# weiquan/salt

Measured on AMD Instinct MI355X. Metric: Mreads/s aligned (100 bp SE, GRCh38+snp144) at 1/2/4/8 MI355X vs CPU ref, higher is better.
Workload: dtype u32; 1 GPU; GRCh38-scale synthetic (SURVEY 8d config 3 = BASELINE configs[2]): 3100000000 bp genome in 24 contigs, 14800000 SNPs, k=21, 1000000 x 100 bp SE reads per GPU per step, 8 distinct resident batches rotated, inputs and results resident in HBM; read_len=100, distinct_batches=8, options=default (-s 50 -m 1000, overlap = k), streams_per_gpu=4

## Files before the change

salt_amd/csrc/salt_align.hip:

```cpp
#include <type_traits>
#include "salt_device.h"
#include "salt_kernels.h"

namespace salt {

#define WSYNC() do { __builtin_amdgcn_fence(__ATOMIC_ACQ_REL, "wavefront"); __builtin_amdgcn_wave_barrier(); \
                     __builtin_amdgcn_fence(__ATOMIC_ACQ_REL, "wavefront"); } while (0)

static constexpr int MAXL = SALT_MAX_READ_LEN;
static constexpr int SLOTS = SALT_MAX_SEED_SLOTS;
static constexpr int MAXLOC = SALT_MAX_LOCATE;
static constexpr int LVK = 31;
static_assert(offsetof(salt_result_t, strand) == 4 && offsetof(salt_result_t, mapq) == 7 && offsetof(salt_result_t, b0) == 8 &&
              offsetof(salt_result_t, b1) == 12 && offsetof(salt_result_t, seq_start) == 16 && offsetof(salt_result_t, seq_end) == 18 &&
              offsetof(salt_result_t, n_hits) == 20 && offsetof(salt_result_t, n_cigar) == 22 && offsetof(salt_result_t, skipped) == 23 &&
              offsetof(salt_result_t, hits) == 24 && sizeof(salt_hit_t) == 8, "salt_result_t header layout");
static constexpr int NHIT = 6;
__device__ __forceinline__ uint32_t mapq_quot(uint32_t x, uint32_t b0)
{
    const uint32_t v = 255u * x;
    return b0 == 1u ? v : b0 == 2u ? v / 2u : b0 == 3u ? v / 3u : v / b0;
}
static constexpr uint32_t INF = 255;

// ... 922 lines not shown
            for (uint32_t k = 0; k < 8; ++k) {
                if (!mm) break;
                const uint32_t bit = (uint32_t)__ffsll((long long)mm) - 1u;
                if (k == q) c = b + bit;
                mm &= mm - 1;
            }
            m = mm;
            const bool act = c != 0xFFFFFFFFu;
            uint32_t pos = act ? cand[c] : 0u;
            if (pos >= ref_len) pos = 0xFFFFFFFFu;
            u32x4_a4 x = { 0u, 0u, 0u, 0u };
            if (act && need && pos != 0xFFFFFFFFu) x = *reinterpret_cast<const u32x4_a4 *>(ref + (pos >> 3) + 4 * sub);
            const uint32_t mism = quad_mismatch<8>(x, pos, pmw, nvalid);
            if (act && sub == 0) out[c] = (uint8_t)((mism > 3 || pos == 0xFFFFFFFFu) ? INF : mism);
        }
    }
}

__device__ __forceinline__ uint32_t popc(uint32_t m) { return (uint32_t)__popc(m); }
__device__ __forceinline__ uint32_t popc(uint64_t m) { return (uint32_t)__popcll(m); }
__device__ __forceinline__ int first_bit(uint32_t m) { return __ffs((int)m) - 1; }
__device__ __forceinline__ int first_bit(uint64_t m) { return __ffsll((long long)m) - 1; }
template <int GW> struct LaneGroup {
    static_assert(GW == 64 || GW == 32, "a wave or half of one");
    typedef std::conditional_t<GW == 64, uint64_t, uint32_t> mask_t;
    static __device__ __forceinline__ uint32_t lane() { return lane_id() & (uint32_t)(GW - 1); }
    static __device__ __forceinline__ mask_t ballot(bool x)
    {
        const uint64_t m = __ballot(x);
        if constexpr (GW == 64) return m; else return (lane_id() & 32u) ? (uint32_t)(m >> 32) : (uint32_t)m;
    }
    static __device__ __forceinline__ uint32_t bcast(uint32_t v, int src)
    {
        if constexpr (GW == 64) return (uint32_t)__builtin_amdgcn_readlane((int)v, src);
        else return (uint32_t)__shfl((int)v, (int)(lane_id() & 32u) + src);
    }
    static __device__ __forceinline__ mask_t below() { return ((mask_t)1 << lane()) - (mask_t)1; }
    static __device__ __forceinline__ uint32_t sum(uint32_t v)
    {
        for (int o = GW / 2; o > 0; o >>= 1) v += (uint32_t)__shfl_xor((int)v, o);
        return v;
    }
};

template <int LN = 4, int GW = 64>
__device__ __forceinline__ void verify_quads_2(const uint32_t *__restrict__ ref, uint32_t ref_len, const uint32_t *pm0, const uint32_t *pm1, uint32_t L,
                                               const uint32_t *c0, uint32_t n0, const uint32_t *c1, uint32_t n1, uint8_t *o0, uint8_t *o1)
{
    constexpr uint32_t CPW = (uint32_t)GW / LN;
    const uint32_t lane = LaneGroup<GW>::lane(), sub = lane & (uint32_t)(LN - 1), q = lane / (uint32_t)LN;
    const uint32_t nw = (L + 7) >> 3, n = n0 + n1;
    const uint32_t nvalid = L > 32u * sub ? (L - 32u * sub < 32u ? L - 32u * sub : 32u) : 0u;
    const bool behind = LN == 8 && GW == 32 && !(4u * sub < nw + 1u);
    uint32_t pa[4], pb[4];
#pragma unroll
    for (int t = 0; t < 4; ++t) { const bool in = (4 * sub + t) < nw; pa[t] = in ? pm0[4 * sub + t] : 0u; pb[t] = in ? pm1[4 * sub + t] : 0u; }
    for (uint32_t b = 0; b < n; b += 4u * CPW) {
        uint32_t pos[4]; u32x4_a4 x[4]; bool act[4], rev[4];
// ... 868 lines not shown
        uint32_t strand, pos, k;
        if (which == 0) { strand = out->strand; pos = out->pos; k = out->n_diff; }
        else {
            const uint32_t h = which - 1, n0 = out->n_hits[0];
            strand = h >= n0; const uint32_t j = strand ? h - n0 : h;
            pos = out->hits[strand][j].pos; k = out->hits[strand][j].n_diff;
        }
        for (uint32_t t = lane; t < (L + 7) >> 3; t += 64) w.pm[strand][t] = rec[strand * ap.pg.nw8 + t];
        WSYNC();
        lv_cigar(ix.ref, w, lvtab + blockIdx.x, (int)strand, L, pos, (int)k);
        uint16_t *dst = which == 0 ? out->cigar : out->hit_cigar[which - 1];
        if (lane < (uint32_t)w.n_cig) dst[lane] = w.cig[lane];
        if (lane == 0) { if (which == 0) out->n_cigar = (uint8_t)w.n_cig; else out->hit_n_cigar[which - 1] = (uint8_t)w.n_cig; }
        WSYNC();
    }
}

__host__ __device__ __forceinline__ uint32_t qseg_cap(uint32_t n_reads) { return n_reads / QUEUE_RANGES + 8u; }
__device__ __forceinline__ void queue_push(uint32_t *__restrict__ qseg, QueueRange *__restrict__ ranges, uint32_t n_reads, uint32_t r)
{
    const uint32_t s = (r >> 2) & (QUEUE_RANGES - 1u);
    qseg[(size_t)s * qseg_cap(n_reads) + atomicAdd(&ranges[s].push, 1u)] = r;
}
__global__ void __launch_bounds__(256)
k_queue_pack(const uint32_t *__restrict__ qseg, const QueueRange *__restrict__ ranges, uint32_t n_reads, uint32_t *__restrict__ queue, SeCtl *__restrict__ ctl)
{
    __shared__ uint32_t base_s, cnt_s;
    if (threadIdx.x == 0) {
        uint32_t base = 0, total = 0;
        for (uint32_t s = 0; s < QUEUE_RANGES; ++s) { const uint32_t c = ranges[s].push; if (s < blockIdx.x) base += c; total += c; }
        base_s = base; cnt_s = ranges[blockIdx.x].push;
        if (blockIdx.x == 0) ctl->light_queued = total;
    }
    __syncthreads();
    const uint32_t *src = qseg + (size_t)blockIdx.x * qseg_cap(n_reads);
    for (uint32_t i = threadIdx.x; i < cnt_s; i += 256) queue[base_s + i] = src[i];
}

static constexpr int LT_LOCI = 128;
static constexpr int LT_MAXL = 160;
static constexpr int L2_SLOTS = 8;

template <int SLOTS, int PMW> struct LightRec {
    uint32_t pm[2][PMW];
    uint32_t sp[4][SLOTS], off[4][SLOTS];
    uint32_t pre[4][SLOTS + 1];
    uint32_t loci[2][LT_LOCI];
    uint32_t hit_pos[2][NHIT];
    uint8_t  hit_nd[2][NHIT];
    uint8_t  val[2][LT_LOCI];
};
template <int GW> using LightLds = LightRec<GW / 4, GW == 64 ? LT_MAXL / 8 : 32>;

template <int GW, int LN, bool INSTR>
__device__ __forceinline__ void light_read(const IndexView &ix, const AlignParams &ap, const uint32_t *__restrict__ pm,
                                           const uint4 *__restrict__ sai_c, const uint4 *__restrict__ sai_r, salt_result_t *__restrict__ results,
                                           uint32_t *__restrict__ queue , QueueRange *__restrict__ ranges,
                                           unsigned long long *__restrict__ ctr, LightLds<GW> &w, const uint32_t r)
{
    typedef LaneGroup<GW> G;
    typedef typename G::mask_t mask_t;
    constexpr uint32_t SLOTS = GW / 4, HALF = GW / 2;
    constexpr uint32_t LMAX = LN == 4 ? 120u : LN == 8 ? 248u : (uint32_t)LT_MAXL;
    static_assert(LMAX <= 8 * sizeof(w.pm[0]) / 4 && (LN != 0 || LMAX <= 248u), "the read fits the record and the window check");
    const uint32_t lane = G::lane();
    const mask_t lt = G::below();
    const uint32_t *rec = pm + (uint64_t)r * ap.pg.pm_stride;
    const uint32_t L = rec[2 * ap.pg.nw8];
    bool heavy = L > LMAX || L < (uint32_t)ap.l_seed || ap.spr > SLOTS || ap.max_locate < 2 * 64;
    uint32_t c_sa_c = 0, c_sa_r = 0, c_verify = 0, c_loci = 0;
    const bool prof = INSTR && ctr && (r & 127u) == 0;
    uint64_t tp = prof ? __builtin_amdgcn_s_memtime() : 0;
    auto stamp = [&](int slot) {
        if (!prof) return;
        const uint64_t n = __builtin_amdgcn_s_memtime();
// ... 30 lines not shown
        uint32_t tot[4];
        bool small;
        {
            const uint32_t l = lane / SLOTS, slot = lane % SLOTS;
            uint4 v = make_uint4(1, 0, 0, 0);
            if (slot < ap.spr) { v = ((l & 1) ? sai_r : sai_c)[((uint64_t)r * 2u + (l >> 1)) * ap.spr + slot]; if (l & 1) v = sai_r_row(v, ap.epoch); }
            uint32_t sz = v.w ? v.y - v.x + 1u : 0u;
            if (sz > 65u) sz = 65u;
            uint32_t inc = sz;
            for (int o = 1; o < (int)SLOTS; o <<= 1) { const uint32_t t = (uint32_t)__shfl_up((int)inc, o, SLOTS); if (slot >= (uint32_t)o) inc += t; }
            for (int q = 0; q < 4; ++q) tot[q] = G::bcast(inc, (int)SLOTS * q + (int)SLOTS - 1);
            small = tot[0] <= SLOTS && tot[1] <= SLOTS && tot[2] <= SLOTS && tot[3] <= SLOTS;
            if (small) {
                for (uint32_t k2 = 0; k2 < sz; ++k2) { w.sp[l][inc - sz + k2] = v.x + k2; w.off[l][inc - sz + k2] = v.z | (v.w == 2 ? 0x80000000u : 0u); }
            } else {
                w.sp[l][slot] = v.x; w.off[l][slot] = v.z | (v.w == 2 ? 0x80000000u : 0u);
                w.pre[l][slot + 1] = inc;
                if (slot == 0) w.pre[l][0] = 0;
            }
        }
        WSYNC();
        stamp(SALT_CTR_LT_SEEDS);
        for (int l = 0; l < 4; ++l) heavy |= tot[l] > 64;
        if (INSTR && ap.dbg_stop == 1) { if (lane == 0) results[r].pos = tot[0] + tot[1] + tot[2] + tot[3] + w.pm[0][0] + w.pm[1][1]; return; }
        if (!heavy) {
            uint32_t n_s[2] = { 0, 0 };
            if (small) {
                const uint32_t l = lane / SLOTS, x = lane % SLOTS;
                const uint32_t tl = l == 0 ? tot[0] : l == 1 ? tot[1] : l == 2 ? tot[2] : tot[3];
                bool keep = false; uint32_t p = 0;
                if (x < tl) keep = locate(l, w.sp[l][x], w.off[l][x], p);
                stamp(SALT_CTR_LT_LOCATE);
                if (INSTR && ap.dbg_stop == 2) { if (__ballot(p == 12345u) == 1) results[r].pos = p; return; }
                const mask_t km = G::ballot(keep);
                const uint32_t k0 = (uint32_t)(km & (((mask_t)1 << HALF) - 1)), k1 = (uint32_t)(km >> HALF), s = lane / HALF;
                if (keep) w.loci[s][popc((s ? k1 : k0) & ((1u << (lane % HALF)) - 1u))] = p;
                n_s[0] = popc(k0); n_s[1] = popc(k1);
                c_sa_c += tot[0] + tot[2]; c_sa_r += tot[1] + tot[3];
            } else {
                auto locate_row = [&](uint32_t l, uint32_t x, uint32_t &p) -> bool {
                    uint32_t i = 0;
                    while (w.pre[l][i + 1] <= x) ++i;
                    return locate(l, w.sp[l][i] + (x - w.pre[l][i]), w.off[l][i], p);
                };
                if constexpr (GW == 64) {
                    uint32_t pos4[4]; bool keep4[4];
                    for (int l = 0; l < 4; ++l) {
                        keep4[l] = false; pos4[l] = 0;
                        if (lane < tot[l]) keep4[l] = locate_row(l, lane, pos4[l]);
                    }
                    stamp(SALT_CTR_LT_LOCATE);
                    if (INSTR && ap.dbg_stop == 2) { const uint32_t x = pos4[0] + pos4[1] + pos4[2] + pos4[3]; if (__ballot(x == 12345u) == 1) results[r].pos = x; return; }
                    for (int s = 0; s < 2; ++s) {
                        const mask_t mc = G::ballot(keep4[2 * s]), mr = G::ballot(keep4[2 * s + 1]);
                        const uint32_t nc = popc(mc);
                        if (keep4[2 * s]) w.loci[s][popc(mc & lt)] = pos4[2 * s];
                        if (keep4[2 * s + 1]) w.loci[s][nc + popc(mr & lt)] = pos4[2 * s + 1];
                        n_s[s] = nc + popc(mr);
                    }
                } else {
                    for (int l = 0; l < 4; ++l) {
                        const int s = l >> 1;
                        for (uint32_t x = lane; x - lane < tot[l]; x += GW) {
                            bool keep = false; uint32_t p = 0;
                            if (x < tot[l]) keep = locate_row(l, x, p);
                            const mask_t km = G::ballot(keep);
                            if (keep) w.loci[s][n_s[s] + popc(km & lt)] = p;
                            n_s[s] += popc(km);
// ... 32 lines not shown
                    cand = hp != 0xFFFFFFFFu && hp != q_pos && (hs ? a0[1] : a0[0]) <= q_ndiff;
                }
                const mask_t cm = G::ballot(cand);
                const bool sel = cand && popc(cm & lt) < (uint32_t)ap.max_hits;
                const mask_t sm = G::ballot(sel);
                const uint32_t nh0 = popc(sm & (((mask_t)1 << NHIT) - 1)), nh1 = popc(sm >> NHIT);
                const int b0 = (int)q_ndiff;
                int b1 = 100000;
                if (nh0) b1 = (int)a0[0];
                if (nh1 && (int)a0[1] <= b1) b1 = (int)a0[1];
                uint32_t mapq = 0;
                if (b0 != 0) {
                    const uint32_t x = (uint32_t)(b0 > b1 ? b0 - b1 : b1 - b0);
                    const uint64_t q = mapq_quot(x, (uint32_t)b0);
                    mapq = q < 254 ? (uint32_t)q : 254u;
                }
                salt_result_t *out = results + r;
                if (sel) {
                    const uint32_t hidx = popc(sm & lt);
                    salt_hit_t hv; hv.pos = hp; hv.n_diff = (uint8_t)hn; hv.is_gap = 0; hv.strand = (uint16_t)hs;
                    out->hits[hs][hs ? hidx - nh0 : hidx] = hv;
                    out->hit_n_cigar[hidx] = 0;
                }
                const uint32_t t = lane - (GW == 64 ? 0u : 16u);
                if (t < 6) {
                    const uint32_t d = t == 0 ? q_pos
                                     : t == 1 ? (q_strand | (q_ndiff << 8) | (mapq << 24))
                                     : t == 2 ? (uint32_t)b0
                                     : t == 3 ? (uint32_t)b1
                                     : t == 4 ? ((L - 1) << 16)
                                     : (nh0 | (nh1 << 8) | (1u << 16));
                    reinterpret_cast<uint32_t *>(out)[t] = d;
                } else if (t == 6) out->cigar[0] = (uint16_t)((L << 4) | 0u);
            }
        }
    }
    if (heavy) {
        if (lane == 0) queue_push(queue, ranges, ap.n_reads, r);
        return;
    }
    if constexpr (INSTR) {
        stamp(SALT_CTR_LT_OUT);
        if (prof && lane == 0) atomicAdd(ctr + SALT_CTR_LT_SAMPLES, 1ull);
        if (ctr && lane == 0) {
            atomicAdd(ctr + SALT_CTR_SA_C, c_sa_c); atomicAdd(ctr + SALT_CTR_SA_R, c_sa_r);
            atomicAdd(ctr + SALT_CTR_VERIFY, c_verify);
            atomicAdd(ctr + SALT_CTR_READS, 1ull); atomicAdd(ctr + SALT_CTR_BASES, L); atomicAdd(ctr + SALT_CTR_LOCI, c_loci);
// ... 5 lines not shown
}

static constexpr int LT_WAVES = 2;
__global__ void __launch_bounds__(64 * LT_WAVES) __attribute__((amdgpu_waves_per_eu(8, 8)))
k_light(IndexView ix, AlignParams ap, const uint32_t *__restrict__ pm,
        const uint4 *__restrict__ sai_c, const uint4 *__restrict__ sai_r, salt_result_t *__restrict__ results,
        uint32_t *__restrict__ queue , QueueRange *__restrict__ ranges, unsigned long long *__restrict__ ctr)
{
    __shared__ LightLds<64> w[LT_WAVES];
    const uint32_t r = __builtin_amdgcn_readfirstlane(blockIdx.x * LT_WAVES + (threadIdx.x >> 6));
    if (r < ap.n_reads) light_read<64, 0, true>(ix, ap, pm, sai_c, sai_r, results, queue, ranges, ctr, w[threadIdx.x >> 6], r);
}

template <int L2_WAVES, int LN = 4>
__global__ void __launch_bounds__(64 * L2_WAVES) __attribute__((amdgpu_waves_per_eu(8, 8)))
k_light2(IndexView ix, AlignParams ap, const uint32_t *__restrict__ pm,
         const uint4 *__restrict__ sai_c, const uint4 *__restrict__ sai_r, salt_result_t *__restrict__ results,
         uint32_t *__restrict__ queue , QueueRange *__restrict__ ranges)
{
    __shared__ LightLds<32> w[2 * L2_WAVES];
    const uint32_t h = 2u * (threadIdx.x >> 6) + (lane_id() >> 5);
    const uint32_t r = 2u * blockIdx.x * (uint32_t)L2_WAVES + h;
    if (r < ap.n_reads) light_read<32, LN, false>(ix, ap, pm, sai_c, sai_r, results, queue, ranges, nullptr, w[h], r);
}

__global__ void __launch_bounds__(256)
k_pe_final(PackGeom pg, uint32_t n_pairs, const uint32_t *__restrict__ pm,
           salt_result_t *__restrict__ res, const PePair *__restrict__ pairs, const PeSwRes *__restrict__ sw,
           uint32_t *__restrict__ citems, uint32_t *__restrict__ ccount)
{
    const uint32_t p = blockIdx.x * blockDim.x + threadIdx.x;
    if (p >= n_pairs) return;
    const PePair pr = pairs[p];
    int rescued = -1;
    for (int k = 0; k < pr.n_req && rescued < 0; ++k) {
        const PeSwRes &r = sw[pr.req0 + k];
        if (!r.ok) continue;
        rescued = pr.rescued[k];
        salt_result_t *q = res + 2 * p + rescued;
        const int b0 = r.score1, b1 = r.score2;
        uint32_t mapq = 0;
        if (b0 != 0) { const uint32_t x = (uint32_t)(b0 > b1 ? b0 - b1 : b1 - b0); const uint64_t v = mapq_quot(x, (uint32_t)b0); mapq = v < 254 ? (uint32_t)v : 254u; }
        q->b0 = b0; q->b1 = b1; q->mapq = (uint8_t)mapq;
        q->pos = (uint32_t)r.ref_begin + r.start; q->strand = (uint8_t)r.strand;
        q->seq_start = (uint16_t)r.read_begin; q->seq_end = (uint16_t)r.read_end;
        q->n_cigar = (uint8_t)r.n_cigar;
// ... 19 lines not shown
}

uint32_t seed_wq_seg_cap(uint64_t items) { return (uint32_t)(((items + 255) / 256 + WQ_SEG - 1) / WQ_SEG) * 256u; }
size_t seed_wq_words(uint64_t items) { return (size_t)2 * WQ_SEG * seed_wq_seg_cap(items) * WQ_REC * 4; }
uint32_t seed_wq_cnt_words() { return 2u * WQ_SEG * WQ_STRIDE; }
void launch_seed(const IndexView &ix, const SeedParams &sp, const uint32_t *tb, uint4 *sai_c, uint4 *sai_r, uint4 *wq, uint32_t *wq_cnt,
                 uint32_t walk_blocks, unsigned long long *ctr, hipStream_t st)
{
    uint64_t items = (uint64_t)sp.n_reads * 2u * sp.spr;
    if (!items) return;
    uint32_t blocks = (uint32_t)((items + 255) / 256);
    const uint32_t cap = seed_wq_seg_cap(items);
    hipLaunchKernelGGL(k_seed, dim3(blocks), dim3(256), 0, st, ix, sp, tb, sai_c, sai_r, wq, wq_cnt, cap, ctr);
    walk_blocks = (walk_blocks + WQ_SEG - 1) / WQ_SEG * WQ_SEG;
    static const uint32_t r_first = getenv("SALT_GPU_WALK_R_FIRST") && atoi(getenv("SALT_GPU_WALK_R_FIRST")) ? 1u : 0u;
    hipLaunchKernelGGL(k_seed_walk, dim3(walk_blocks), dim3(256), 0, st, ix, sp, tb, sai_c, sai_r, wq, wq_cnt, cap, r_first, ctr);
}

void launch_light(const IndexView &ix, const AlignParams &ap, const uint32_t *pm, const uint8_t *, const uint32_t *, const uint4 *sai_c,
                  const uint4 *sai_r, salt_result_t *results, uint32_t *queue, SeCtl *ctl, uint32_t *qseg, QueueRange *ranges, unsigned long long *ctr, hipStream_t st)
{
    if (!ap.n_reads) return;
    static const bool no_half = getenv("SALT_GPU_NO_LIGHT2") && atoi(getenv("SALT_GPU_NO_LIGHT2"));
    if (!no_half && !ctr && !SALT_DIAG_VAL(ap.dbg_stop) && ap.spr <= (uint32_t)L2_SLOTS && ap.pg.nw8 <= 31) {
        static const int wv = getenv("SALT_GPU_L2_WAVES") ? atoi(getenv("SALT_GPU_L2_WAVES")) : 2;
        if (ap.pg.nw8 > 15) hipLaunchKernelGGL((k_light2<2, 8>), dim3((ap.n_reads + 3) / 4), dim3(128), 0, st, ix, ap, pm, sai_c, sai_r, results, qseg, ranges);
        else if (wv == 1) hipLaunchKernelGGL(k_light2<1>, dim3((ap.n_reads + 1) / 2), dim3(64), 0, st, ix, ap, pm, sai_c, sai_r, results, qseg, ranges);
        else hipLaunchKernelGGL(k_light2<2>, dim3((ap.n_reads + 3) / 4), dim3(128), 0, st, ix, ap, pm, sai_c, sai_r, results, qseg, ranges);
    } else
        hipLaunchKernelGGL(k_light, dim3((ap.n_reads + LT_WAVES - 1) / LT_WAVES), dim3(64 * LT_WAVES), 0, st, ix, ap, pm, sai_c, sai_r, results, qseg, ranges, ctr);
    hipLaunchKernelGGL(k_queue_pack, dim3(QUEUE_RANGES), dim3(256), 0, st, qseg, ranges, ap.n_reads, queue, ctl);
}
size_t queue_words(uint32_t max_reads) { return (size_t)max_reads * 2 + (size_t)QUEUE_RANGES * qseg_cap(max_reads); }

__global__ void __launch_bounds__(64)
k_diag_rule(uint32_t n_cases, const uint32_t *__restrict__ pos, const uint8_t *__restrict__ val, const uint32_t *__restrict__ offs,
            const uint32_t *__restrict__ bound_in, uint32_t L, uint32_t ref_len, int mode, uint32_t *__restrict__ out)
{
    __shared__ uint32_t hit_pos_s[2][NHIT];
    __shared__ uint8_t hit_nd_s[2][NHIT];
    const uint32_t half = mode == 3 ? lane_id() >> 5 : 0u, lane = mode == 3 ? lane_id() & 31u : lane_id();
    const uint32_t c = mode == 3 ? 2u * blockIdx.x + half : blockIdx.x;
    if (c >= n_cases) return;
    uint32_t *hit_pos = hit_pos_s[half];
    uint8_t *hit_nd = hit_nd_s[half];
    const uint32_t o = offs[c], n = offs[c + 1] - o;
    uint32_t bound = bound_in[c], bp = 0, bv = 0, nh = 0, a0 = 0;
    bool any = false;
    if (lane < NHIT) { hit_pos[lane] = 0; hit_nd[lane] = 0; }
    WSYNC();
    if (mode == 0) rule_unsorted<3, false>(pos + o, val + o, n, L, ref_len, bound, any, bp, bv, nh, a0, hit_pos, hit_nd);
    else if (mode == 1) rule_sparse<3, false>(pos + o, val + o, n, L, ref_len, bound, any, bp, bv, nh, a0, hit_pos, hit_nd);
    else if (mode == 3) rule_sparse<3, false, 32>(pos + o, val + o, n, L, ref_len, bound, any, bp, bv, nh, a0, hit_pos, hit_nd);
    else rule_unsorted<LLV_K, true>(pos + o, val + o, n, L, ref_len, bound, any, bp, bv, nh, a0, hit_pos, hit_nd);
    WSYNC();
    uint32_t *w = out + (size_t)c * (6 + 2 * NHIT);
    if (lane == 0) { w[0] = any; w[1] = any ? bp : 0; w[2] = any ? bv : 0; w[3] = nh; w[4] = nh ? a0 : 0; w[5] = bound; }
    if (lane < NHIT) { w[6 + 2 * lane] = lane < nh ? hit_pos[lane] : 0; w[7 + 2 * lane] = lane < nh ? hit_nd[lane] : 0; }
}

void launch_diag_rule(uint32_t n_cases, const uint32_t *pos, const uint8_t *val, const uint32_t *offs, const uint32_t *bound_in,
                      uint32_t L, uint32_t ref_len, int mode, uint32_t *out, hipStream_t st)
{
    const uint32_t blocks = mode == 3 ? (n_cases + 1) / 2 : n_cases;
    if (n_cases) hipLaunchKernelGGL(k_diag_rule, dim3(blocks), dim3(64), 0, st, n_cases, pos, val, offs, bound_in, L, ref_len, mode, out);
}
uint32_t diag_rule_words() { return 6 + 2 * NHIT; }

__host__ __device__ static inline bool lv_fit_dev(uint32_t L, uint32_t k) { return k <= (uint32_t)LLV_K && L + 4 <= 8u * (LLV_TW - 1); }
bool lv_lanes_fit(uint32_t L, uint32_t k) { return lv_fit_dev(L, k); }

__global__ void __launch_bounds__(64)
k_diag_lv(IndexView ix, uint32_t n_cases, const uint32_t *__restrict__ pos, const uint32_t *__restrict__ kdiff,
          const uint8_t *__restrict__ seqs, const uint32_t *__restrict__ offs, const uint32_t *__restrict__ lane_first,
          const uint32_t *__restrict__ lane_n, const uint32_t *__restrict__ lane_case, int32_t *__restrict__ out ,
          uint16_t *__restrict__ cig_out , LvTables *__restrict__ lvtab)
{
    __shared__ WaveLds w;
    __shared__ uint32_t lane_pm[LLV_N][LLV_PW];
    const uint32_t c = blockIdx.x, lane = lane_id();
    if (c >= n_cases) return;
    const uint32_t off = offs[c], L = offs[c + 1] - off, p = pos[c];
    const uint32_t nw = (L + 7) >> 3;
    auto pm_word = [&](uint32_t o, uint32_t j) -> uint32_t {
        uint32_t word = 0;
        for (uint32_t q = 0; q < 8; ++q) {
            uint32_t i = j * 8 + q, cc = i < L ? seqs[o + i] : 5u;
// ... 30 lines not shown
        n_cig = w.n_cig;
        if (lane < (uint32_t)w.n_cig) cig_out[(size_t)c * SALT_MAX_CIGAR_OPS + lane] = w.cig[lane];
    }
    if (lane == 0) {
        out[(size_t)c * 4 + 0] = v; out[(size_t)c * 4 + 1] = e_wave; out[(size_t)c * 4 + 3] = n_cig;
        if (!fit) out[(size_t)c * 4 + 2] = -2;
    }
}

size_t lv_table_bytes() { return sizeof(LvTables); }

void launch_diag_lv(const IndexView &ix, uint32_t n, const uint32_t *pos, const uint32_t *kdiff, const uint8_t *seqs,
                    const uint32_t *offs, const uint32_t *lane_first, const uint32_t *lane_n, const uint32_t *lane_case,
                    int32_t *out, uint16_t *cig, void *lvtab, hipStream_t st)
{
    if (n) hipLaunchKernelGGL(k_diag_lv, dim3(n), dim3(64), 0, st, ix, n, pos, kdiff, seqs, offs, lane_first, lane_n, lane_case, out, cig,
                              static_cast<LvTables *>(lvtab));
}

__global__ void __launch_bounds__(64)
k_diag_verify(const uint32_t *__restrict__ ref, uint32_t ref_len, uint32_t n_cases, const uint8_t *__restrict__ seqs, const uint32_t *__restrict__ offs,
              const uint32_t *__restrict__ cand, const uint32_t *__restrict__ coffs, int mode, uint8_t *__restrict__ out)
{
    __shared__ uint32_t pm_s[2][64];
    __shared__ uint32_t loci_s[2][256];
    __shared__ uint8_t val_s[2][256];
    const uint32_t gw = mode >= 5 ? 32u : 64u, half = mode >= 5 ? lane_id() >> 5 : 0u, lane = lane_id() & (gw - 1u);
    const uint32_t c = mode >= 5 ? 2u * blockIdx.x + half : blockIdx.x;
    if (c >= n_cases) return;
    uint32_t *pm = pm_s[half], *loci = loci_s[half];
    uint8_t *val = val_s[half];
    const uint32_t off = offs[c], L = offs[c + 1] - off, c0 = coffs[c];
    uint32_t n = coffs[c + 1] - c0;
    if (n > 256) n = 256;
    const uint32_t nw = (L + 7) >> 3;
    for (uint32_t j = lane; j < 64; j += gw) {
        uint32_t word = 0;
        for (uint32_t q = 0; q < 8 && j < nw; ++q) {
            const uint32_t i = j * 8 + q, cc = i < L ? seqs[off + i] : 5u;
            word |= (cc < 4 ? (1u << cc) : (cc == 4 ? 15u : 0u)) << (4 * q);
        }
        pm[j] = word;
    }
    for (uint32_t i = lane; i < n; i += gw) { loci[i] = cand[c0 + i]; val[i] = 77; }
    WSYNC();
    IndexView ix; ix.ref = ref; ix.ref_len = ref_len;
    if (mode == 0) { for (uint32_t i = lane; i < n; i += 64) val[i] = (uint8_t)mismatch_capped(ix, pm, L, loci[i]); }
    else if (mode == 1) verify_quads<8>(ref, ref_len, pm, L, loci, n, val);
    else if (mode == 2) verify_quads<8, 8>(ref, ref_len, pm, L, loci, n, val);
    else if (mode == 3) verify_quads_2(ref, ref_len, pm, pm, L, loci, n / 2, loci + n / 2, n - n / 2, val, val + n / 2);
    else if (mode == 4) verify_quads_2<8>(ref, ref_len, pm, pm, L, loci, n / 2, loci + n / 2, n - n / 2, val, val + n / 2);
    else if (mode == 5) verify_quads_2<4, 32>(ref, ref_len, pm, pm, L, loci, n / 2, loci + n / 2, n - n / 2, val, val + n / 2);
    else verify_quads_2<8, 32>(ref, ref_len, pm, pm, L, loci, n / 2, loci + n / 2, n - n / 2, val, val + n / 2);
    WSYNC();
    for (uint32_t i = lane; i < n; i += gw) out[c0 + i] = val[i];
}
void launch_diag_verify(const uint32_t *ref, uint32_t ref_len, uint32_t n_cases, const uint8_t *seqs, const uint32_t *offs, const uint32_t *cand,
                        const uint32_t *coffs, int mode, uint8_t *out, hipStream_t st)
{
    const uint32_t blocks = mode >= 5 ? (n_cases + 1) / 2 : n_cases;
    if (n_cases) hipLaunchKernelGGL(k_diag_verify, dim3(blocks), dim3(64), 0, st, ref, ref_len, n_cases, seqs, offs, cand, coffs, mode, out);
}

__global__ void __launch_bounds__(64)
k_polish(const uint8_t *__restrict__ pac, const uint8_t *__restrict__ codes, const uint32_t *__restrict__ offs, const salt_polish_item_t *__restrict__ items,
         uint32_t n_items, const uint8_t *__restrict__ pool, uint32_t pool_stride, int want_cigar, int32_t *__restrict__ dist,
         uint16_t *__restrict__ cigars, uint8_t *__restrict__ n_cigar, LvTables *__restrict__ tabs)
{
    __shared__ LvBytes s;
    __shared__ int s_n;
    const uint32_t lane = lane_id();
    for (uint32_t it = blockIdx.x; it < n_items; it += gridDim.x) {
        const salt_polish_item_t x = items[it];
        const uint32_t o = offs[x.read], L = offs[x.read + 1] - o, tl = x.tlen;
        WSYNC();
        for (uint32_t i = lane; i < L + 48; i += 64) {
            uint8_t pv = 1;
            if (i < L) { const uint8_t c = x.strand ? codes[o + L - 1 - i] : codes[o + i]; pv = c < 4 ? (uint8_t)(1u << (x.strand ? 3 - c : c)) : (uint8_t)(x.strand ? 0x20 : 0x10); }
            s.P[i] = pv;
        }
        for (uint32_t i = lane; i < L + 48; i += 64) {
            uint8_t tv = 1;
            if (x.pool != 0xFFFFFFFFu) { if (i < pool_stride) tv = (uint8_t)(1u << (pool[(uint64_t)x.pool * pool_stride + i] & 3u)); }
// ... 137 lines not shown
```

salt_amd/csrc/salt_gpu.hip:

```cpp
#include <hip/hip_runtime.h>
#include <stdio.h>
#include <stdlib.h>
#include <string.h>
#include <time.h>
#include <cstddef>
#include <cctype>
#include <map>
#include <utility>
#include <string>
#include <thread>
#include <vector>
#include <algorithm>
#include "salt_kernels.h"
#include "salt_inflate_block.h"
#include <rccl/rccl.h>

using namespace salt;

static thread_local std::string g_err;
static int fail(int code, const std::string &msg) { g_err = msg; return code; }

#define HIPCHK(x) do { hipError_t e_ = (x); if (e_ != hipSuccess) \
    return fail(SALT_E_HIP, std::string(#x) + ": " + hipGetErrorString(e_)); } while (0)
#define DONECHK(x) do { hipError_t e_ = (x); if (e_ != hipSuccess) return done(fail(SALT_E_HIP, std::string(#x) + ": " + hipGetErrorString(e_))); } while (0)
// ... 1501 lines not shown
    if (n == 0) return SALT_OK;
    const uint32_t hi = mode == 0 ? ix->hdr.c_seq_len : ix->hdr.r_text_len + 1, n_sym = mode == 0 ? 4u : 5u;
    for (uint32_t i = 0; i < n; ++i) {
        const uint32_t *q = queries + 3 * (uint64_t)i;
        for (int e = 0; e < 2; ++e) if (q[e] > hi && !(mode == 0 && q[e] == 0xFFFFFFFFu)) return fail(SALT_E_INVAL, "query " + std::to_string(i) + ": index outside the primitive's range");
        if (q[2] >= n_sym) return fail(SALT_E_INVAL, "query " + std::to_string(i) + ": symbol outside the alphabet");
    }
    HIPCHK(hipSetDevice(ix->device));
    uint32_t *d_q = nullptr, *d_out = nullptr;
    auto done = [&](int rc) { hipFree(d_q); hipFree(d_out); return rc; };
    DONECHK(hipMalloc((void **)&d_q, (uint64_t)n * 12)); DONECHK(hipMemcpy(d_q, queries, (uint64_t)n * 12, hipMemcpyHostToDevice));
    DONECHK(hipMalloc((void **)&d_out, (uint64_t)n * 48));
    launch_diag_occ(ix->view, mode, n, d_q, d_out, nullptr);
    DONECHK(hipGetLastError());
    DONECHK(hipDeviceSynchronize());
    DONECHK(hipMemcpy(out, d_out, (uint64_t)n * 48, hipMemcpyDeviceToHost));
    return done(SALT_OK);
}

extern "C" int salt_gpu_diag_verify(const uint32_t *ref_words, uint32_t ref_len, uint32_t n_cases, const uint8_t *seqs, const uint32_t *offs,
                                    const uint32_t *cand, const uint32_t *cand_offs, int mode, uint8_t *out)
{
    if (!ref_words || !seqs || !offs || !cand || !cand_offs || !out) return fail(SALT_E_INVAL, "null argument");
    if (mode < 0 || mode > 6) return fail(SALT_E_INVAL, "mode must be 0..6");
    if (n_cases == 0) return SALT_OK;
    int n_dev = 0;
    HIPCHK(hipGetDeviceCount(&n_dev));
    if (n_dev <= 0) return fail(SALT_E_HIP, "no HIP device visible");
    for (uint32_t i = 0; i < n_cases; ++i) {
        const uint32_t L = offs[i + 1] - offs[i];
        if (L == 0 || L > SALT_MAX_READ_LEN || ((mode == 1 || mode == 3 || mode == 5) && L > 120) || ((mode == 2 || mode == 4 || mode == 6) && L > 248)) return fail(SALT_E_INVAL, "read length outside the verifier's range");
        if (cand_offs[i + 1] - cand_offs[i] > 256) return fail(SALT_E_INVAL, "at most 256 candidates per case");
    }
    const uint64_t nw = ((uint64_t)ref_len + 7) / 8 + 36, bases = offs[n_cases], nc = cand_offs[n_cases];
    uint32_t *d_ref = nullptr, *d_offs = nullptr, *d_cand = nullptr, *d_coffs = nullptr; uint8_t *d_seqs = nullptr, *d_out = nullptr;
    HIPCHK(hipMalloc((void **)&d_ref, nw * 4)); HIPCHK(hipMemset(d_ref, 0, nw * 4));
    HIPCHK(hipMemcpy(d_ref, ref_words, (nw - 36) * 4, hipMemcpyHostToDevice));
    HIPCHK(hipMalloc((void **)&d_offs, ((uint64_t)n_cases + 1) * 4)); HIPCHK(hipMemcpy(d_offs, offs, ((uint64_t)n_cases + 1) * 4, hipMemcpyHostToDevice));
    HIPCHK(hipMalloc((void **)&d_coffs, ((uint64_t)n_cases + 1) * 4)); HIPCHK(hipMemcpy(d_coffs, cand_offs, ((uint64_t)n_cases + 1) * 4, hipMemcpyHostToDevice));
    HIPCHK(hipMalloc((void **)&d_cand, (nc + 1) * 4)); HIPCHK(hipMemcpy(d_cand, cand, nc * 4, hipMemcpyHostToDevice));
    HIPCHK(hipMalloc((void **)&d_seqs, bases + 64)); HIPCHK(hipMemcpy(d_seqs, seqs, bases, hipMemcpyHostToDevice));
    HIPCHK(hipMalloc((void **)&d_out, nc + 1));
    launch_diag_verify(d_ref, ref_len, n_cases, d_seqs, d_offs, d_cand, d_coffs, mode, d_out, nullptr);
    HIPCHK(hipGetLastError());
    HIPCHK(hipDeviceSynchronize());
    HIPCHK(hipMemcpy(out, d_out, nc, hipMemcpyDeviceToHost));
    hipFree(d_ref); hipFree(d_offs); hipFree(d_coffs); hipFree(d_cand); hipFree(d_seqs); hipFree(d_out);
    return SALT_OK;
}

extern "C" int salt_gpu_ws_queue_counts(salt_gpu_ws_t *ws, uint32_t out[8])
{
    if (!ws || !out) return fail(SALT_E_INVAL, "null argument");
    HIPCHK(hipSetDevice(ws->ix->device));
    HIPCHK(hipDeviceSynchronize());
    SeCtl c; HIPCHK(hipMemcpy(&c, ws->d_qctl, sizeof c, hipMemcpyDeviceToHost));
    memset(out, 0, 32);
    out[0] = c.light_queued; out[2] = c.gap_slots; out[5] = c.gap_items; out[6] = c.cigar_items; out[7] = c.cigar_head;
    {
        std::vector<uint32_t> wc(seed_wq_cnt_words());
        HIPCHK(hipMemcpy(wc.data(), ws->d_wq_cnt, wc.size() * 4, hipMemcpyDeviceToHost));
        const uint32_t per_list = seed_wq_cnt_words() / 2u, stride = per_list / 64u;
        for (uint32_t i = 0; i < 64u; ++i) { out[1] = std::max(out[1], wc[i * stride]); out[3] = std::max(out[3], wc[per_list + i * stride]); }
    }
    return SALT_OK;
}

extern "C" int salt_gpu_ws_heavy_reads(salt_gpu_ws_t *ws, uint32_t *ids, uint32_t cap, uint32_t *n)
{
    if (!ws || !n) return fail(SALT_E_INVAL, "null argument");
    HIPCHK(hipSetDevice(ws->ix->device));
    HIPCHK(hipDeviceSynchronize());
    HIPCHK(hipMemcpy(n, &ws->d_qctl->light_queued, 4, hipMemcpyDeviceToHost));
    if (ids && cap) HIPCHK(hipMemcpy(ids, ws->d_queue, (uint64_t)(*n < cap ? *n : cap) * 4, hipMemcpyDeviceToHost));
    return SALT_OK;
}

extern "C" int salt_gpu_index_set_pac(salt_gpu_index_t *ix, const uint8_t *pac, uint64_t l_pac)
{
    if (!ix || !pac || l_pac == 0) return fail(SALT_E_INVAL, "null argument");
    HIPCHK(hipSetDevice(ix->device));
// ... 344 lines not shown
```

salt_amd/csrc/salt_kernels.h:

```cpp
#pragma once
#include <hip/hip_runtime.h>
#include <cstddef>
#include <string>
#include <vector>
#include "../../include/salt_gpu.h"
#include "salt_device.h"

#ifdef SALT_DIAG
#define SALT_DIAG_VAL(x) (x)
#else
#define SALT_DIAG_VAL(x) 0
#endif

namespace salt {

struct PackGeom {
    uint32_t nw8, nw16, nw32, pm_stride, tb_stride;
    __host__ __device__ static PackGeom make(uint32_t max_len)
    {
        if (max_len < 1) max_len = 1;
        PackGeom g; g.nw8 = (max_len + 7) / 8; g.nw16 = (max_len + 15) / 16; g.nw32 = (max_len + 31) / 32;
        g.pm_stride = (2 * g.nw8 + 1 + 3) & ~3u; g.tb_stride = (2 * g.nw16 + 2 * g.nw32 + 1 + 3) & ~3u;
        return g;
    }
// ... 28 lines not shown
void launch_seed(const IndexView &ix, const SeedParams &sp, const uint32_t *tb, uint4 *sai_c, uint4 *sai_r, uint4 *wq, uint32_t *wq_cnt,
                 uint32_t walk_blocks, unsigned long long *ctr, hipStream_t st);
size_t seed_wq_words(uint64_t items);
uint32_t seed_wq_cnt_words();
__device__ __forceinline__ uint32_t sw_pull(uint32_t *head, const uint32_t step, const uint32_t n_first, const uint32_t n_items)
{
    if (n_first >= n_items || n_first + __hip_atomic_load(head, __ATOMIC_RELAXED, __HIP_MEMORY_SCOPE_AGENT) >= n_items) return 0xFFFFFFFFu;
    return n_first + atomicAdd(head, step);
}
struct SeCtl {
    alignas(128) uint32_t light_queued;
    alignas(128) uint32_t gap_slots;
    alignas(128) uint32_t gap_items;
    alignas(128) uint32_t cigar_items;
    alignas(128) uint32_t cigar_head;
    alignas(128) uint32_t pool_used;
    alignas(128) uint32_t ovq_count;
    alignas(128) uint32_t ovq_head;
};
static_assert(sizeof(SeCtl) == 8 * 128 && alignof(SeCtl) == 128, "one control word per 128-byte line");
static const uint32_t QUEUE_RANGES = 64;
struct QueueRange {
    enum { HEAVY, GAP, GAPFIN };
    uint32_t push, pad0[31], heads[3], pad1[29];
};
static_assert(sizeof(QueueRange) == 256 && offsetof(QueueRange, push) == 0 && offsetof(QueueRange, heads) == 128, "k_light's counter, then the heads");
void launch_light(const IndexView &ix, const AlignParams &ap, const uint32_t *pm, const uint8_t *seqs, const uint32_t *offs, const uint4 *sai_c,
                  const uint4 *sai_r, salt_result_t *results, uint32_t *queue, SeCtl *ctl, uint32_t *qseg, QueueRange *ranges, unsigned long long *ctr, hipStream_t st);
size_t queue_words(uint32_t max_reads);
struct GapBufs {
    uint32_t *gq;
    uint32_t *gn;
    uint32_t *goff;
    uint32_t *gloci;
    uint8_t  *ge;
    uint32_t *gitems;
    uint32_t *cq;
    SeCtl *gctl;
    uint32_t cap, pool, items_cap;
    uint32_t *ovq;
    QueueRange *ranges;
};
GapBufs gap_bufs_layout(uint8_t *base, uint32_t cap, SeCtl *gctl, size_t *bytes);
void launch_heavy(const IndexView &ix, const AlignParams &ap, const uint32_t *pm, const uint4 *sai_c,
                  const uint4 *sai_r, salt_result_t *results, const uint32_t *queue, unsigned long long *ctr,
                  uint32_t n_blocks, uint32_t gap_blocks, void *lvtab, const GapBufs &g, uint32_t *ovq, QueueRange *ranges, uint8_t *pe_scr, hipEvent_t *ev3, hipStream_t st);
size_t lv_table_bytes();
// ... 141 lines not shown
```

Before: 522.7 Mreads/s.

## Add quarter-wave light-read kernel with half-wave retry for overflow reads

Adds a k_light4 path that processes four reads per wavefront (16 lanes each) with smaller LDS records. It is selected by default when seeds per read are at most 4 and reads fit 120 bp. Reads whose per-seed hit count exceeds the 16-row capacity are pushed to a new retry queue, and a persistent half-wave kernel reprocesses them. The aim is more reads in flight and less lane idling for short, low-hit reads. The cost is a second launch, retry overhead and narrower lanes for seed and verify work. The queue buffer doubles to hold the retry segments, and the diagnostic kernels gain 16-lane modes.

```diff
diff --git a/salt_amd/csrc/salt_align.hip b/salt_amd/csrc/salt_align.hip
--- a/salt_amd/csrc/salt_align.hip
+++ b/salt_amd/csrc/salt_align.hip
@@ -968,18 +968,22 @@
 __device__ __forceinline__ int first_bit(uint32_t m) { return __ffs((int)m) - 1; }
 __device__ __forceinline__ int first_bit(uint64_t m) { return __ffsll((long long)m) - 1; }
 template <int GW> struct LaneGroup {
-    static_assert(GW == 64 || GW == 32, "a wave or half of one");
+    static_assert(GW == 64 || GW == 32 || GW == 16, "a wave, half of one or a quarter");
     typedef std::conditional_t<GW == 64, uint64_t, uint32_t> mask_t;
     static __device__ __forceinline__ uint32_t lane() { return lane_id() & (uint32_t)(GW - 1); }
     static __device__ __forceinline__ mask_t ballot(bool x)
     {
         const uint64_t m = __ballot(x);
-        if constexpr (GW == 64) return m; else return (lane_id() & 32u) ? (uint32_t)(m >> 32) : (uint32_t)m;
+        if constexpr (GW == 64) return m;
+        else {
+            const uint32_t h = (lane_id() & 32u) ? (uint32_t)(m >> 32) : (uint32_t)m;
+            if constexpr (GW == 32) return h; else return (h >> (lane_id() & 16u)) & 0xFFFFu;
+        }
     }
     static __device__ __forceinline__ uint32_t bcast(uint32_t v, int src)
     {
         if constexpr (GW == 64) return (uint32_t)__builtin_amdgcn_readlane((int)v, src);
-        else return (uint32_t)__shfl((int)v, (int)(lane_id() & 32u) + src);
+        else return (uint32_t)__shfl((int)v, (int)(lane_id() & (uint32_t)(64 - GW)) + src);
     }
     static __device__ __forceinline__ mask_t below() { return ((mask_t)1 << lane()) - (mask_t)1; }
     static __device__ __forceinline__ uint32_t sum(uint32_t v)
@@ -1894,6 +1898,12 @@
     const uint32_t s = (r >> 2) & (QUEUE_RANGES - 1u);
     qseg[(size_t)s * qseg_cap(n_reads) + atomicAdd(&ranges[s].push, 1u)] = r;
 }
+__device__ __forceinline__ uint32_t *retry_segs(uint32_t *qseg, uint32_t n_reads) { return qseg + (size_t)QUEUE_RANGES * qseg_cap(n_reads); }
+__device__ __forceinline__ void retry_push(uint32_t *__restrict__ qseg, QueueRange *__restrict__ ranges, uint32_t n_reads, uint32_t r)
+{
+    const uint32_t s = (r >> 2) & (QUEUE_RANGES - 1u);
+    retry_segs(qseg, n_reads)[(size_t)s * qseg_cap(n_reads) + atomicAdd(&ranges[s].retry, 1u)] = r;
+}
 __global__ void __launch_bounds__(256)
 k_queue_pack(const uint32_t *__restrict__ qseg, const QueueRange *__restrict__ ranges, uint32_t n_reads, uint32_t *__restrict__ queue, SeCtl *__restrict__ ctl)
 {
@@ -1912,17 +1922,23 @@
 static constexpr int LT_LOCI = 128;
 static constexpr int LT_MAXL = 160;
 static constexpr int L2_SLOTS = 8;
-
-template <int SLOTS, int PMW> struct LightRec {
+static constexpr int L4_SLOTS = 4;
+#ifndef SALT_L4_ROWS
+#define SALT_L4_ROWS 16
+#endif
+static constexpr int L4_ROWS = SALT_L4_ROWS;
+
+template <int SLOTS, int PMW, int LOCI> struct LightRec {
     uint32_t pm[2][PMW];
     uint32_t sp[4][SLOTS], off[4][SLOTS];
     uint32_t pre[4][SLOTS + 1];
-    uint32_t loci[2][LT_LOCI];
+    uint32_t loci[2][LOCI];
     uint32_t hit_pos[2][NHIT];
     uint8_t  hit_nd[2][NHIT];
-    uint8_t  val[2][LT_LOCI];
+    uint8_t  val[2][LOCI];
 };
-template <int GW> using LightLds = LightRec<GW / 4, GW == 64 ? LT_MAXL / 8 : 32>;
+template <int GW> using LightLds = LightRec<GW / 4, GW == 64 ? LT_MAXL / 8 : GW == 32 ? 32 : 16, GW == 16 ? 2 * L4_ROWS : LT_LOCI>;
+static_assert(sizeof(LightLds<32>) == 1996 && 8 * sizeof(LightLds<16>) <= 4 * sizeof(LightLds<32>), "eight quarter records in the LDS of four half-wave ones");
 
 template <int GW, int LN, bool INSTR>
 __device__ __forceinline__ void light_read(const IndexView &ix, const AlignParams &ap, const uint32_t *__restrict__ pm,
@@ -1999,6 +2015,12 @@
         WSYNC();
         stamp(SALT_CTR_LT_SEEDS);
         for (int l = 0; l < 4; ++l) heavy |= tot[l] > 64;
+        if constexpr (GW == 16) {
+            if (!heavy && (tot[0] > (uint32_t)L4_ROWS || tot[1] > (uint32_t)L4_ROWS || tot[2] > (uint32_t)L4_ROWS || tot[3] > (uint32_t)L4_ROWS)) {
+                if (lane == 0) retry_push(queue, ranges, ap.n_reads, r);
+                return;
+            }
+        }
         if (INSTR && ap.dbg_stop == 1) { if (lane == 0) results[r].pos = tot[0] + tot[1] + tot[2] + tot[3] + w.pm[0][0] + w.pm[1][1]; return; }
         if (!heavy) {
             uint32_t n_s[2] = { 0, 0 };
@@ -2020,7 +2042,7 @@
                     while (w.pre[l][i + 1] <= x) ++i;
                     return locate(l, w.sp[l][i] + (x - w.pre[l][i]), w.off[l][i], p);
                 };
-                if constexpr (GW == 64) {
+                if constexpr (GW == 64 || (GW == 16 && L4_ROWS <= 16)) {
                     uint32_t pos4[4]; bool keep4[4];
                     for (int l = 0; l < 4; ++l) {
                         keep4[l] = false; pos4[l] = 0;
@@ -2099,7 +2121,7 @@
                     out->hits[hs][hs ? hidx - nh0 : hidx] = hv;
                     out->hit_n_cigar[hidx] = 0;
                 }
-                const uint32_t t = lane - (GW == 64 ? 0u : 16u);
+                const uint32_t t = lane - (GW == 32 ? 16u : 0u);
                 if (t < 6) {
                     const uint32_t d = t == 0 ? q_pos
                                      : t == 1 ? (q_strand | (q_ndiff << 8) | (mapq << 24))
@@ -2151,6 +2173,34 @@
     const uint32_t h = 2u * (threadIdx.x >> 6) + (lane_id() >> 5);
     const uint32_t r = 2u * blockIdx.x * (uint32_t)L2_WAVES + h;
     if (r < ap.n_reads) light_read<32, LN, false>(ix, ap, pm, sai_c, sai_r, results, queue, ranges, nullptr, w[h], r);
+}
+
+template <int L4_WAVES>
+__global__ void __launch_bounds__(64 * L4_WAVES) __attribute__((amdgpu_waves_per_eu(8, 8)))
+k_light4(IndexView ix, AlignParams ap, const uint32_t *__restrict__ pm,
+         const uint4 *__restrict__ sai_c, const uint4 *__restrict__ sai_r, salt_result_t *__restrict__ results,
+         uint32_t *__restrict__ queue , QueueRange *__restrict__ ranges)
+{
+    __shared__ LightLds<16> w[4 * L4_WAVES];
+    const uint32_t q = 4u * (threadIdx.x >> 6) + (lane_id() >> 4);
+    const uint32_t r = 4u * blockIdx.x * (uint32_t)L4_WAVES + q;
+    if (r < ap.n_reads) light_read<16, 4, false>(ix, ap, pm, sai_c, sai_r, results, queue, ranges, nullptr, w[q], r);
+}
+
+__global__ void __launch_bounds__(128)
+k_light_retry(IndexView ix, AlignParams ap, const uint32_t *__restrict__ pm,
+              const uint4 *__restrict__ sai_c, const uint4 *__restrict__ sai_r, salt_result_t *__restrict__ results,
+              uint32_t *__restrict__ queue , QueueRange *__restrict__ ranges)
+{
+    __shared__ LightLds<32> w[4];
+    const uint32_t h = 2u * (threadIdx.x >> 6) + (lane_id() >> 5);
+    const uint32_t seg = blockIdx.x & (QUEUE_RANGES - 1u), step = 4u * (gridDim.x / QUEUE_RANGES);
+    const uint32_t cnt = __hip_atomic_load(&ranges[seg].retry, __ATOMIC_RELAXED, __HIP_MEMORY_SCOPE_AGENT);
+    const uint32_t *src = retry_segs(queue, ap.n_reads) + (size_t)seg * qseg_cap(ap.n_reads);
+    for (uint32_t i = 4u * (blockIdx.x / QUEUE_RANGES) + h; i < cnt; i += step) {
+        light_read<32, 4, false>(ix, ap, pm, sai_c, sai_r, results, queue, ranges, nullptr, w[h], src[i]);
+        WSYNC();
+    }
 }
 
 __global__ void __launch_bounds__(256)
@@ -2216,7 +2266,20 @@
 {
     if (!ap.n_reads) return;
     static const bool no_half = getenv("SALT_GPU_NO_LIGHT2") && atoi(getenv("SALT_GPU_NO_LIGHT2"));
-    if (!no_half && !ctr && !SALT_DIAG_VAL(ap.dbg_stop) && ap.spr <= (uint32_t)L2_SLOTS && ap.pg.nw8 <= 31) {
+    static const bool no_quarter = getenv("SALT_GPU_NO_LIGHT4") && atoi(getenv("SALT_GPU_NO_LIGHT4"));
+    if (!no_half && !no_quarter && !ctr && !SALT_DIAG_VAL(ap.dbg_stop) && ap.spr <= (uint32_t)L4_SLOTS && ap.pg.nw8 <= 15) {
+        static const int wv = getenv("SALT_GPU_L4_WAVES") ? atoi(getenv("SALT_GPU_L4_WAVES")) : 2;
+        if (wv == 1) hipLaunchKernelGGL(k_light4<1>, dim3((ap.n_reads + 3) / 4), dim3(64), 0, st, ix, ap, pm, sai_c, sai_r, results, qseg, ranges);
+        else if (wv == 4) hipLaunchKernelGGL(k_light4<4>, dim3((ap.n_reads + 15) / 16), dim3(256), 0, st, ix, ap, pm, sai_c, sai_r, results, qseg, ranges);
+        else hipLaunchKernelGGL(k_light4<2>, dim3((ap.n_reads + 7) / 8), dim3(128), 0, st, ix, ap, pm, sai_c, sai_r, results, qseg, ranges);
+        static const uint32_t retry_blocks = [] {
+            int dev = 0, cus = 0, per_cu = getenv("SALT_GPU_L4_RETRY_PER_CU") ? atoi(getenv("SALT_GPU_L4_RETRY_PER_CU")) : 8;
+            if (hipGetDevice(&dev) != hipSuccess || hipDeviceGetAttribute(&cus, hipDeviceAttributeMultiprocessorCount, dev) != hipSuccess || cus <= 0) cus = (int)QUEUE_RANGES;
+            if (per_cu < 1 || per_cu > 64) per_cu = 8;
+            return ((uint32_t)(cus * per_cu) + QUEUE_RANGES - 1u) / QUEUE_RANGES * QUEUE_RANGES;
+        }();
+        hipLaunchKernelGGL(k_light_retry, dim3(retry_blocks), dim3(128), 0, st, ix, ap, pm, sai_c, sai_r, results, qseg, ranges);
+    } else if (!no_half && !ctr && !SALT_DIAG_VAL(ap.dbg_stop) && ap.spr <= (uint32_t)L2_SLOTS && ap.pg.nw8 <= 31) {
         static const int wv = getenv("SALT_GPU_L2_WAVES") ? atoi(getenv("SALT_GPU_L2_WAVES")) : 2;
         if (ap.pg.nw8 > 15) hipLaunchKernelGGL((k_light2<2, 8>), dim3((ap.n_reads + 3) / 4), dim3(128), 0, st, ix, ap, pm, sai_c, sai_r, results, qseg, ranges);
         else if (wv == 1) hipLaunchKernelGGL(k_light2<1>, dim3((ap.n_reads + 1) / 2), dim3(64), 0, st, ix, ap, pm, sai_c, sai_r, results, qseg, ranges);
@@ -2225,16 +2288,16 @@
         hipLaunchKernelGGL(k_light, dim3((ap.n_reads + LT_WAVES - 1) / LT_WAVES), dim3(64 * LT_WAVES), 0, st, ix, ap, pm, sai_c, sai_r, results, qseg, ranges, ctr);
     hipLaunchKernelGGL(k_queue_pack, dim3(QUEUE_RANGES), dim3(256), 0, st, qseg, ranges, ap.n_reads, queue, ctl);
 }
-size_t queue_words(uint32_t max_reads) { return (size_t)max_reads * 2 + (size_t)QUEUE_RANGES * qseg_cap(max_reads); }
+size_t queue_words(uint32_t max_reads) { return (size_t)max_reads * 2 + (size_t)2 * QUEUE_RANGES * qseg_cap(max_reads); }
 
 __global__ void __launch_bounds__(64)
 k_diag_rule(uint32_t n_cases, const uint32_t *__restrict__ pos, const uint8_t *__restrict__ val, const uint32_t *__restrict__ offs,
             const uint32_t *__restrict__ bound_in, uint32_t L, uint32_t ref_len, int mode, uint32_t *__restrict__ out)
 {
-    __shared__ uint32_t hit_pos_s[2][NHIT];
-    __shared__ uint8_t hit_nd_s[2][NHIT];
-    const uint32_t half = mode == 3 ? lane_id() >> 5 : 0u, lane = mode == 3 ? lane_id() & 31u : lane_id();
-    const uint32_t c = mode == 3 ? 2u * blockIdx.x + half : blockIdx.x;
+    __shared__ uint32_t hit_pos_s[4][NHIT];
+    __shared__ uint8_t hit_nd_s[4][NHIT];
+    const uint32_t gw = mode == 3 ? 32u : mode == 4 ? 16u : 64u, half = lane_id() / gw, lane = lane_id() & (gw - 1u);
+    const uint32_t c = (64u / gw) * blockIdx.x + half;
     if (c >= n_cases) return;
     uint32_t *hit_pos = hit_pos_s[half];
     uint8_t *hit_nd = hit_nd_s[half];
@@ -2246,6 +2309,7 @@
     if (mode == 0) rule_unsorted<3, false>(pos + o, val + o, n, L, ref_len, bound, any, bp, bv, nh, a0, hit_pos, hit_nd);
     else if (mode == 1) rule_sparse<3, false>(pos + o, val + o, n, L, ref_len, bound, any, bp, bv, nh, a0, hit_pos, hit_nd);
     else if (mode == 3) rule_sparse<3, false, 32>(pos + o, val + o, n, L, ref_len, bound, any, bp, bv, nh, a0, hit_pos, hit_nd);
+    else if (mode == 4) rule_sparse<3, false, 16>(pos + o, val + o, n, L, ref_len, bound, any, bp, bv, nh, a0, hit_pos, hit_nd);
     else rule_unsorted<LLV_K, true>(pos + o, val + o, n, L, ref_len, bound, any, bp, bv, nh, a0, hit_pos, hit_nd);
     WSYNC();
     uint32_t *w = out + (size_t)c * (6 + 2 * NHIT);
@@ -2256,7 +2320,7 @@
 void launch_diag_rule(uint32_t n_cases, const uint32_t *pos, const uint8_t *val, const uint32_t *offs, const uint32_t *bound_in,
                       uint32_t L, uint32_t ref_len, int mode, uint32_t *out, hipStream_t st)
 {
-    const uint32_t blocks = mode == 3 ? (n_cases + 1) / 2 : n_cases;
+    const uint32_t blocks = mode == 3 ? (n_cases + 1) / 2 : mode == 4 ? (n_cases + 3) / 4 : n_cases;
     if (n_cases) hipLaunchKernelGGL(k_diag_rule, dim3(blocks), dim3(64), 0, st, n_cases, pos, val, offs, bound_in, L, ref_len, mode, out);
 }
 uint32_t diag_rule_words() { return 6 + 2 * NHIT; }
@@ -2333,11 +2397,11 @@
 k_diag_verify(const uint32_t *__restrict__ ref, uint32_t ref_len, uint32_t n_cases, const uint8_t *__restrict__ seqs, const uint32_t *__restrict__ offs,
               const uint32_t *__restrict__ cand, const uint32_t *__restrict__ coffs, int mode, uint8_t *__restrict__ out)
 {
-    __shared__ uint32_t pm_s[2][64];
-    __shared__ uint32_t loci_s[2][256];
-    __shared__ uint8_t val_s[2][256];
-    const uint32_t gw = mode >= 5 ? 32u : 64u, half = mode >= 5 ? lane_id() >> 5 : 0u, lane = lane_id() & (gw - 1u);
-    const uint32_t c = mode >= 5 ? 2u * blockIdx.x + half : blockIdx.x;
+    __shared__ uint32_t pm_s[4][64];
+    __shared__ uint32_t loci_s[4][256];
+    __shared__ uint8_t val_s[4][256];
+    const uint32_t gw = mode == 7 ? 16u : mode >= 5 ? 32u : 64u, half = lane_id() / gw, lane = lane_id() & (gw - 1u);
+    const uint32_t c = (64u / gw) * blockIdx.x + half;
     if (c >= n_cases) return;
     uint32_t *pm = pm_s[half], *loci = loci_s[half];
     uint8_t *val = val_s[half];
@@ -2362,14 +2426,15 @@
     else if (mode == 3) verify_quads_2(ref, ref_len, pm, pm, L, loci, n / 2, loci + n / 2, n - n / 2, val, val + n / 2);
     else if (mode == 4) verify_quads_2<8>(ref, ref_len, pm, pm, L, loci, n / 2, loci + n / 2, n - n / 2, val, val + n / 2);
     else if (mode == 5) verify_quads_2<4, 32>(ref, ref_len, pm, pm, L, loci, n / 2, loci + n / 2, n - n / 2, val, val + n / 2);
-    else verify_quads_2<8, 32>(ref, ref_len, pm, pm, L, loci, n / 2, loci + n / 2, n - n / 2, val, val + n / 2);
+    else if (mode == 6) verify_quads_2<8, 32>(ref, ref_len, pm, pm, L, loci, n / 2, loci + n / 2, n - n / 2, val, val + n / 2);
+    else verify_quads_2<4, 16>(ref, ref_len, pm, pm, L, loci, n / 2, loci + n / 2, n - n / 2, val, val + n / 2);
     WSYNC();
     for (uint32_t i = lane; i < n; i += gw) out[c0 + i] = val[i];
 }
 void launch_diag_verify(const uint32_t *ref, uint32_t ref_len, uint32_t n_cases, const uint8_t *seqs, const uint32_t *offs, const uint32_t *cand,
                         const uint32_t *coffs, int mode, uint8_t *out, hipStream_t st)
 {
-    const uint32_t blocks = mode >= 5 ? (n_cases + 1) / 2 : n_cases;
+    const uint32_t blocks = mode == 7 ? (n_cases + 3) / 4 : mode >= 5 ? (n_cases + 1) / 2 : n_cases;
     if (n_cases) hipLaunchKernelGGL(k_diag_verify, dim3(blocks), dim3(64), 0, st, ref, ref_len, n_cases, seqs, offs, cand, coffs, mode, out);
 }
 
diff --git a/salt_amd/csrc/salt_gpu.hip b/salt_amd/csrc/salt_gpu.hip
--- a/salt_amd/csrc/salt_gpu.hip
+++ b/salt_amd/csrc/salt_gpu.hip
@@ -1547,14 +1547,14 @@
                                     const uint32_t *cand, const uint32_t *cand_offs, int mode, uint8_t *out)
 {
     if (!ref_words || !seqs || !offs || !cand || !cand_offs || !out) return fail(SALT_E_INVAL, "null argument");
-    if (mode < 0 || mode > 6) return fail(SALT_E_INVAL, "mode must be 0..6");
+    if (mode < 0 || mode > 7) return fail(SALT_E_INVAL, "mode must be 0..7");
     if (n_cases == 0) return SALT_OK;
     int n_dev = 0;
     HIPCHK(hipGetDeviceCount(&n_dev));
     if (n_dev <= 0) return fail(SALT_E_HIP, "no HIP device visible");
     for (uint32_t i = 0; i < n_cases; ++i) {
         const uint32_t L = offs[i + 1] - offs[i];
-        if (L == 0 || L > SALT_MAX_READ_LEN || ((mode == 1 || mode == 3 || mode == 5) && L > 120) || ((mode == 2 || mode == 4 || mode == 6) && L > 248)) return fail(SALT_E_INVAL, "read length outside the verifier's range");
+        if (L == 0 || L > SALT_MAX_READ_LEN || ((mode == 1 || mode == 3 || mode == 5 || mode == 7) && L > 120) || ((mode == 2 || mode == 4 || mode == 6) && L > 248)) return fail(SALT_E_INVAL, "read length outside the verifier's range");
         if (cand_offs[i + 1] - cand_offs[i] > 256) return fail(SALT_E_INVAL, "at most 256 candidates per case");
     }
     const uint64_t nw = ((uint64_t)ref_len + 7) / 8 + 36, bases = offs[n_cases], nc = cand_offs[n_cases];
@@ -1582,6 +1582,11 @@
     SeCtl c; HIPCHK(hipMemcpy(&c, ws->d_qctl, sizeof c, hipMemcpyDeviceToHost));
     memset(out, 0, 32);
     out[0] = c.light_queued; out[2] = c.gap_slots; out[5] = c.gap_items; out[6] = c.cigar_items; out[7] = c.cigar_head;
+    {
+        std::vector<QueueRange> qr(QUEUE_RANGES);
+        HIPCHK(hipMemcpy(qr.data(), ws->d_ranges, qr.size() * sizeof(QueueRange), hipMemcpyDeviceToHost));
+        for (const QueueRange &q : qr) out[4] += q.retry;
+    }
     {
         std::vector<uint32_t> wc(seed_wq_cnt_words());
         HIPCHK(hipMemcpy(wc.data(), ws->d_wq_cnt, wc.size() * 4, hipMemcpyDeviceToHost));
diff --git a/salt_amd/csrc/salt_kernels.h b/salt_amd/csrc/salt_kernels.h
--- a/salt_amd/csrc/salt_kernels.h
+++ b/salt_amd/csrc/salt_kernels.h
@@ -74,7 +74,7 @@
 static const uint32_t QUEUE_RANGES = 64;
 struct QueueRange {
     enum { HEAVY, GAP, GAPFIN };
-    uint32_t push, pad0[31], heads[3], pad1[29];
+    uint32_t push, pad0[31], heads[3], retry, pad1[28];
 };
 static_assert(sizeof(QueueRange) == 256 && offsetof(QueueRange, push) == 0 && offsetof(QueueRange, heads) == 128, "k_light's counter, then the heads");
 void launch_light(const IndexView &ix, const AlignParams &ap, const uint32_t *pm, const uint8_t *seqs, const uint32_t *offs, const uint4 *sai_c,
```

After: 553.5 Mreads/s (median of 6 runs). 1.06x the previous value.
